# socom20/speech-cloner

Measured on AMD Instinct MI355X. Metric: mel frames/sec, higher is better.
Workload: dtype bf16; 1 GPU; full: STFT+mel front-end on batch 32 x 4 s @ 16 kHz (configs[1] input) -> 64 windows of 400 frames -> encoder (enc_14 weights) + decoder (hp/decoder_cfg_d.json sizes, random init), 64 windows per launch, independent steps pipelined over 10 HIP streams; batch=32, samples=64000, windows=64, model_dtype=bfloat16, streams=10, parallelism=utterance-sharded x1, no collective

## Files before the change

### include/vc_hip.h

```cpp
#ifndef VC_HIP_H
#define VC_HIP_H

#include <stddef.h>
#include <stdint.h>

#ifdef __cplusplus
extern "C" {
#endif

#define VC_OK 0
#define VC_ERR_INVALID 1
#define VC_ERR_HIP 2
#define VC_ERR_WORKSPACE 3
#define VC_ERR_UNSUPPORTED 4

#define VC_ABI_VERSION 7

int vc_version(void);
const char* vc_last_error(void);
const char* vc_target_arch(void);

int vc_set_option(const char* name, int value);
int vc_get_option(const char* name, int* value);

// ... 248 lines not shown
                           vc_vocoder_plan** out_plan);
void vc_vocoder_plan_destroy(vc_vocoder_plan* plan);
int32_t vc_vocoder_num_samples(const vc_vocoder_plan* plan, int32_t n_frames);
size_t vc_vocoder_workspace_bytes(const vc_vocoder_plan* plan, int32_t batch, int32_t max_frames, int32_t trace);

int vc_power_to_amp(const float* d_P, const int32_t* d_n_frames, int32_t batch, int32_t max_frames, int32_t n_bins,
                    float P_dB_norm_factor, float realse, float* d_amp, void* stream);

int vc_griffin_lim_f32(const vc_vocoder_plan* plan, const float* d_amp, const float* d_phase0,
                       const int32_t* d_n_frames, int32_t batch, int32_t max_frames, int32_t num_iters,
                       float* d_wav, int32_t wav_stride, float* d_trace, void* d_workspace, size_t workspace_bytes,
                       void* stream);

size_t vc_vocoder_workspace_bytes_momentum(const vc_vocoder_plan* plan, int32_t batch, int32_t max_frames,
                                           int32_t trace);
int vc_griffin_lim_momentum_f32(const vc_vocoder_plan* plan, const float* d_amp, const float* d_phase0,
                                const int32_t* d_n_frames, int32_t batch, int32_t max_frames, int32_t num_iters,
                                float momentum, float* d_wav, int32_t wav_stride, float* d_trace, void* d_workspace,
                                size_t workspace_bytes, void* stream);

int vc_inv_preemphasis_normalize(const vc_vocoder_plan* plan, float* d_wav, const int32_t* d_n_frames, int32_t batch,
                                 int32_t max_frames, int32_t wav_stride, float coeff, float mean_abs_amp_norm,
                                 void* stream);

int vc_highway_pack(const void* d_Bt, int32_t n_cols, int32_t H, void* d_packed, void* stream);
int vc_highway_chain(const void* d_X, int32_t M, int32_t H, int32_t ldx, int32_t n_layers,
                     const void* const* d_packed, const float* const* d_bias, void* d_Y, int32_t ldy,
                     const void* d_proj_packed, const float* d_proj_bias, int32_t n_proj, float* d_P, int32_t ldp,
                     void* stream);

#define VC_CBHG_FRONT_MAX_HIGHWAY 4
typedef struct vc_cbhg_front_desc {
    const void* d_x;
    int32_t x_f32, ldx;
    int32_t n_windows, T;
    int32_t n_features, prenet_units, width, n_banks, bank_filters, n_highway, gru_units;
    const void *d_pk_dense1, *d_pk_dense2, *d_pk_bank, *d_pk_proj1, *d_pk_proj2, *d_pk_gru;
    const void* d_pk_highway[VC_CBHG_FRONT_MAX_HIGHWAY];
    const float* d_coef;
    float* d_xproj;
    int32_t ldp;
} vc_cbhg_front_desc;
int vc_mfma_pack(const void* d_W, int32_t rows, int32_t K, int32_t ldw, int32_t chained, void* d_packed, void* stream);
int32_t vc_cbhg_front_coef_floats(void);
int vc_cbhg_front_supported(int32_t n_features, int32_t prenet_units, int32_t width, int32_t n_banks,
                            int32_t bank_filters, int32_t n_highway, int32_t gru_units, int32_t T);
int vc_cbhg_front(const vc_cbhg_front_desc* desc, void* stream);

int vc_prenet_chain_supported(int32_t cin_padded, int32_t units1, int32_t units2);
int vc_prenet_chain(const void* d_X, int32_t x_f32, int32_t M, int32_t ldx, int32_t cin_padded, int32_t units1, int32_t units2,
                    const void* d_pk1, const float* d_b1, const void* d_pk2, const float* d_b2, void* d_Y, int32_t ldy,
                    void* stream);

int vc_gather_rows(const void* d_src, const int64_t* d_index, const void* d_pad_row, int64_t n_rows,
                   int32_t row_bytes, void* d_dst, void* stream);

int vc_convert(const void* d_src, int32_t src_dtype, void* d_dst, int32_t dst_dtype, size_t n, void* stream);

int vc_cut_windows(const float* d_src, const int32_t* d_win_tab, const int32_t* d_n_frames, int32_t batch,
                   int32_t max_frames, int32_t n_windows, int32_t T, int32_t C, float* d_dst, void* stream);

int vc_compound_stitch(const void* d_src, int32_t src_dtype, const int32_t* d_utt_tab, int32_t batch, int32_t n_windows,
                       int32_t T, int32_t C, int32_t out_frames, float* d_dst, float* d_amp, float P_dB_norm_factor,
                       void* stream);

int vc_phase_init(const int32_t* d_n_frames, const int32_t* d_utt_id, int32_t batch, int32_t max_frames, int32_t n_bins,
                  int64_t seed, float* d_phase, void* stream);

size_t vc_phase_spsi_workspace_bytes(int32_t batch, int32_t max_frames, int32_t n_bins);
int vc_phase_spsi(const float* d_amp, const int32_t* d_n_frames, int32_t batch, int32_t max_frames, int32_t n_bins,
                  int32_t n_fft, int32_t hop, float* d_phase, void* d_workspace, size_t workspace_bytes, void* stream);

typedef struct vc_resample_plan vc_resample_plan;
int vc_resample_plan_create(int32_t up, int32_t down, int32_t half, const double* h_taps, vc_resample_plan** out_plan);
void vc_resample_plan_destroy(vc_resample_plan* plan);
int vc_resample_f32(const vc_resample_plan* plan, const float* d_in, const int32_t* d_lens_in, int32_t batch, int32_t max_in,
                    int32_t ld_in, float* d_out, int32_t max_out, int32_t ld_out, void* stream);

int vc_mel_cepstra(const void* d_mel, int32_t mel_dtype, int32_t rows, int32_t n_mels, const float* d_dct, int32_t n_coef,
                   float* d_cep, void* stream);
size_t vc_dtw_workspace_size(int32_t batch, int32_t max_a, int32_t max_b, int32_t want_path);
int vc_dtw_f32(const float* d_ca, const float* d_cb, const int32_t* d_len_a, const int32_t* d_len_b, int32_t batch,
               int32_t max_a, int32_t max_b, int32_t n_coef, float scale, int32_t band, int32_t want_path, float* d_total,
               int32_t* d_path_len, float* d_mcd, void* d_workspace, size_t workspace_bytes, void* stream);
int vc_dtw_backtrack(const void* d_workspace, size_t workspace_bytes, const int32_t* d_len_a, const int32_t* d_len_b,
                     const float* d_total, const int32_t* d_path_len, int32_t batch, int32_t max_a, int32_t max_b, int32_t* d_path,
                     void* stream);
int vc_frame_mcd_f32(const float* d_ca, const float* d_cb, const int32_t* d_len_a, const int32_t* d_len_b, int32_t batch,
                     int32_t max_a, int32_t max_b, int32_t n_coef, float scale, float* d_mcd, void* stream);

int vc_f0_yin_f32(const float* d_wav, const int32_t* d_lens, int32_t batch, int32_t max_len, int32_t ld, float sample_rate,
                  int32_t hop, int32_t frame_length, int32_t tau_min, int32_t tau_max, float threshold, float* d_f0,
                  float* d_aperiodicity, int32_t max_frames, void* stream);
int vc_f0_metrics_f32(const float* d_f0_a, const float* d_f0_b, const int32_t* d_len_a, const int32_t* d_len_b, int32_t batch,
                      int32_t max_a, int32_t max_b, const int32_t* d_path, const int32_t* d_path_len, int32_t max_path,
                      int32_t* d_counts, float* d_values, void* stream);

int vc_f0_candidates_f32(const float* d_wav, const int32_t* d_lens, int32_t batch, int32_t max_len, int32_t ld, float sample_rate,
                         int32_t hop, int32_t frame_length, int32_t tau_min, int32_t tau_max, float ceiling, int32_t n_cand,
                         float* d_f0, float* d_pitch, float* d_cost, int32_t* d_n, float* d_aperiodicity, int32_t max_frames,
                         void* stream);
int32_t vc_f0_viterbi_tile(void);
size_t vc_f0_viterbi_workspace_size(int32_t batch, int32_t max_frames, int32_t n_cand);
int vc_f0_viterbi_f32(const float* d_pitch, const float* d_cost, const int32_t* d_n, const int32_t* d_frames, int32_t batch,
                      int32_t max_frames, int32_t n_cand, float unvoiced_cost, float jump_cost, float switch_cost,
                      const float* d_cand_f0, int32_t* d_state, float* d_f0, float* d_total, void* d_workspace,
// ... 76 lines not shown
```

### speech-cloner_amd/_vc.py

```python
import contextlib
import ctypes as C
import os
import threading


_HERE = os.path.dirname(os.path.abspath(__file__))
LIB_PATH = os.environ.get('VC_LIB_PATH', os.path.join(_HERE, 'libvc_hip.so'))

VC_OK = 0
VC_ABI_VERSION = 7


class VCError(RuntimeError):
    pass


class FrontendCfg(C.Structure):
    _fields_ = [('sample_rate', C.c_int32), ('hop_length', C.c_int32), ('win_length', C.c_int32),
                ('n_fft', C.c_int32), ('n_mels', C.c_int32), ('n_mfcc', C.c_int32),
                ('pre_emphasis', C.c_float), ('mean_abs_amp_norm', C.c_float),
                ('mfcc_norm_factor', C.c_float), ('M_dB_norm_factor', C.c_float),
                ('P_dB_norm_factor', C.c_float),
                ('mfcc_normaleze_first_mfcc', C.c_int32), ('calc_mfcc_derivate', C.c_int32),
                ('clip_output', C.c_int32)]
# ... 118 lines not shown
    'vc_conv_gemm_workspace_bytes': (C.c_size_t, [C.POINTER(GemmDesc)]),
    'vc_conv_gemm': (C.c_int, [C.POINTER(GemmDesc), _P]),
    'vc_softmax_argmax': (C.c_int, [_P, C.c_int32, C.c_int32, C.c_int32, _P, C.c_int32, C.c_int32, _P, _P]),
    'vc_softmax_argmax_dual': (C.c_int, [_P, C.c_int32, C.c_int32, C.c_int32, _P, C.c_int32, _P, C.c_int32, _P, _P]),
    'vc_gru_workspace_bytes': (C.c_size_t, [C.c_int32, C.c_int32]),
    'vc_gru_bidir': (C.c_int, [_P, _P, _P, C.c_int32, C.c_int32, C.c_int32, C.c_int32, _P, C.c_int32, _P,
                               C.c_size_t, _P]),
    'vc_gru_form': (C.c_int32, [C.c_int32] * 4),
    'vc_gru_packed_bytes': (C.c_size_t, [C.c_int32] * 3),
    'vc_gru_pack': (C.c_int, [C.c_int32, _P, _P, C.c_int32, C.c_int32, _P, C.c_size_t, _P]),
    'vc_gru_bidir_packed': (C.c_int, [C.c_int32, _P, _P, C.c_size_t, C.c_int32, C.c_int32, C.c_int32, C.c_int32, _P, C.c_int32, _P]),
    'vc_lstm_bidir': (C.c_int, [_P, _P, _P, C.c_int32, C.c_int32, C.c_int32, C.c_int32, _P, C.c_int32, _P]),
    'vc_convert': (C.c_int, [_P, C.c_int32, _P, C.c_int32, C.c_size_t, _P]),
    'vc_conv_wgrad': (C.c_int, [C.POINTER(WgradDesc), _P]),
    'vc_transpose_pad': (C.c_int, [_P, C.c_int32, C.c_int32, C.c_int32, C.c_int32, _P, _P, C.c_int32, C.c_int32,
                                   C.c_int32, _P, C.c_int32, C.c_int32, C.c_int32, _P]),
    'vc_stats_workspace_floats': (C.c_size_t, [C.c_int32, C.c_int32]),
    'vc_bn_train_stats': (C.c_int, [_P, C.c_int32, C.c_int32, C.c_int32, _P, _P, _P, _P, C.c_float, C.c_float,
                                    _P, _P, _P, _P, _P, _P]),
    'vc_affine_act': (C.c_int, [_P, _P, _P, C.c_int32, _P, _P, C.c_size_t, C.c_int32, _P]),
    'vc_bn_backward': (C.c_int, [_P, _P, C.c_int32, C.c_int32, C.c_int32, C.c_int32, _P, _P, _P, _P, _P,
                                 C.c_int32, _P, _P, _P, _P, _P]),
    'vc_lstm_train_forward': (C.c_int, [_P, _P, _P, C.c_int32, C.c_int32, C.c_int32, _P, _P, _P, _P]),
    'vc_lstm_backward': (C.c_int, [_P, _P, _P, _P, _P, C.c_int32, C.c_int32, C.c_int32, _P, _P]),
    'vc_bn_post_routing': (C.c_int, [_P, C.c_int32, C.c_int32, C.c_int32, C.c_int32, _P, _P, _P, _P]),
    'vc_relu_dropout_backward': (C.c_int, [_P, _P, C.c_float, _P, C.c_size_t, _P]),
    'vc_highway_backward': (C.c_int, [_P, C.c_int32, _P, _P, C.c_int32, C.c_int32, _P, _P, _P]),
    'vc_col_sum': (C.c_int, [_P, C.c_int32, C.c_int32, C.c_int32, _P, C.c_int32, _P, _P]),
    'vc_fill': (C.c_int, [_P, C.c_float, C.c_size_t, _P]),
    'vc_weight_layouts': (C.c_int, [_P, C.c_int32, _P]),
    'vc_split16': (C.c_int, [_P, C.c_int32, C.c_int32, C.c_int32, C.c_int32, _P, _P, C.c_int32, C.c_int32, _P, _P, _P]),
    'vc_weights16': (C.c_int, [_P, C.c_int32, _P, C.c_int32, _P]),
    'vc_transpose_split16': (C.c_int, [_P, C.c_int32, C.c_int32, C.c_int32, C.c_int32, _P, _P, C.c_int32, C.c_int32, C.c_int32,
                                       C.c_int32, _P, _P, _P]),
    'vc_gemm16_workspace_bytes': (C.c_size_t, [C.c_int32, C.c_int32, C.c_int32]),
    'vc_gemm16': (C.c_int, [C.POINTER(Gemm16Desc), _P]),
    'vc_mx8_quantize': (C.c_int, [_P, C.c_int32, C.c_int32, C.c_int32, C.c_int32, _P, _P, _P]),
    'vc_mx8_conv_workspace_bytes': (C.c_size_t, [C.POINTER(Mx8ConvDesc)]),
    'vc_mx8_conv': (C.c_int, [C.POINTER(Mx8ConvDesc), _P]),
    'vc_axpby': (C.c_int, [_P, C.c_int32, C.c_float, _P, C.c_int32, C.c_float, _P, C.c_int32, C.c_int32, C.c_int32, _P]),
    'vc_mse_loss': (C.c_int, [_P, _P, C.c_size_t, C.c_float, _P, C.c_int32, C.c_int32, _P, _P, _P]),
    'vc_softmax_ce': (C.c_int, [_P, _P, C.c_int32, C.c_int32, C.c_int32, _P, C.c_int32, _P, _P, _P]),
    'vc_adam_step': (C.c_int, [_P, _P, _P, _P, C.c_size_t, C.c_float, C.c_float, C.c_float, C.c_float,
                               C.c_float, _P]),
    'vc_gru_train_forward': (C.c_int, [_P, _P, _P, C.c_int32, C.c_int32, C.c_int32, _P, _P, _P, _P]),
    'vc_gru_backward': (C.c_int, [_P, _P, _P, _P, _P, _P, _P, C.c_int32, C.c_int32, C.c_int32, _P, _P]),
    'vc_conv_gemm_epi_pool_supported': (C.c_int, [C.POINTER(GemmDesc)]),
    'vc_highway_pack': (C.c_int, [_P, C.c_int32, C.c_int32, _P, _P]),
    'vc_highway_chain': (C.c_int, [_P, C.c_int32, C.c_int32, C.c_int32, C.c_int32, C.POINTER(_P), C.POINTER(_P), _P, C.c_int32,
                                   _P, _P, C.c_int32, _P, C.c_int32, _P]),
    'vc_mfma_pack': (C.c_int, [_P, C.c_int32, C.c_int32, C.c_int32, C.c_int32, _P, _P]),
    'vc_prenet_chain_supported': (C.c_int, [C.c_int32] * 3),
    'vc_prenet_chain': (C.c_int, [_P, C.c_int32, C.c_int32, C.c_int32, C.c_int32, C.c_int32, C.c_int32, _P, _P, _P, _P, _P, C.c_int32, _P]),
    'vc_cbhg_front_coef_floats': (C.c_int32, []),
    'vc_cbhg_front_supported': (C.c_int, [C.c_int32] * 8),
    'vc_cbhg_front': (C.c_int, [C.POINTER(CbhgFrontDesc), _P]),
    'vc_gather_rows': (C.c_int, [_P, _P, _P, C.c_int64, C.c_int32, _P, _P]),
    'vc_vocoder_plan_create': (C.c_int, [C.c_int32, C.c_int32, C.c_int32, _P, C.POINTER(_P)]),
    'vc_vocoder_plan_destroy': (None, [_P]),
    'vc_vocoder_num_samples': (C.c_int32, [_P, C.c_int32]),
    'vc_vocoder_workspace_bytes': (C.c_size_t, [_P, C.c_int32, C.c_int32, C.c_int32]),
    'vc_power_to_amp': (C.c_int, [_P, _P, C.c_int32, C.c_int32, C.c_int32, C.c_float, C.c_float, _P, _P]),
    'vc_griffin_lim_f32': (C.c_int, [_P, _P, _P, _P, C.c_int32, C.c_int32, C.c_int32, _P, C.c_int32, _P, _P,
                                     C.c_size_t, _P]),
    'vc_vocoder_workspace_bytes_momentum': (C.c_size_t, [_P, C.c_int32, C.c_int32, C.c_int32]),
    'vc_griffin_lim_momentum_f32': (C.c_int, [_P, _P, _P, _P, C.c_int32, C.c_int32, C.c_int32, C.c_float, _P, C.c_int32,
                                              _P, _P, C.c_size_t, _P]),
    'vc_inv_preemphasis_normalize': (C.c_int, [_P, _P, _P, C.c_int32, C.c_int32, C.c_int32, C.c_float, C.c_float, _P]),
    'vc_cut_windows': (C.c_int, [_P, _P, _P, C.c_int32, C.c_int32, C.c_int32, C.c_int32, C.c_int32, _P, _P]),
    'vc_compound_stitch': (C.c_int, [_P, C.c_int32, _P, C.c_int32, C.c_int32, C.c_int32, C.c_int32, C.c_int32, _P, _P,
                                     C.c_float, _P]),
    'vc_phase_init': (C.c_int, [_P, _P, C.c_int32, C.c_int32, C.c_int32, C.c_int64, _P, _P]),
    'vc_phase_spsi_workspace_bytes': (C.c_size_t, [C.c_int32, C.c_int32, C.c_int32]),
    'vc_phase_spsi': (C.c_int, [_P, _P, C.c_int32, C.c_int32, C.c_int32, C.c_int32, C.c_int32, _P, _P, C.c_size_t, _P]),
    'vc_resample_plan_create': (C.c_int, [C.c_int32, C.c_int32, C.c_int32, _P, C.POINTER(_P)]),
    'vc_resample_plan_destroy': (None, [_P]),
    'vc_resample_f32': (C.c_int, [_P, _P, _P, C.c_int32, C.c_int32, C.c_int32, _P, C.c_int32, C.c_int32, _P]),
    'vc_mel_cepstra': (C.c_int, [_P, C.c_int32, C.c_int32, C.c_int32, _P, C.c_int32, _P, _P]),
    'vc_dtw_workspace_size': (C.c_size_t, [C.c_int32] * 4),
    'vc_dtw_f32': (C.c_int, [_P, _P, _P, _P, C.c_int32, C.c_int32, C.c_int32, C.c_int32, C.c_float, C.c_int32, C.c_int32, _P, _P, _P,
                             _P, C.c_size_t, _P]),
    'vc_dtw_backtrack': (C.c_int, [_P, C.c_size_t, _P, _P, _P, _P, C.c_int32, C.c_int32, C.c_int32, _P, _P]),
    'vc_frame_mcd_f32': (C.c_int, [_P, _P, _P, _P, C.c_int32, C.c_int32, C.c_int32, C.c_int32, C.c_float, _P, _P]),
    'vc_frame_energy_tile': (C.c_int, [C.c_int32, C.c_int32]),
    'vc_frame_energy_f32': (C.c_int, [_P, _P, C.c_int32, C.c_int32, C.c_int32, C.c_int32, C.c_int32, _P, C.c_int32, _P]),
    'vc_activity_mask': (C.c_int, [_P, _P, _P, C.c_int32, C.c_int32, C.c_int32, C.c_float, C.c_int32, C.c_int32, _P, _P]),
    'vc_mask_compact': (C.c_int, [_P, _P, C.c_int32, _P, _P, C.c_int32, C.c_int32, _P, _P, _P, _P, _P, _P]),
    'vc_compact_rows_f32': (C.c_int, [_P, C.c_int32, _P, C.c_int32, _P, C.c_int32, C.c_int32, _P, C.c_int32, _P]),
    'vc_path_map': (C.c_int, [_P, _P, C.c_int32, C.c_int32, _P, C.c_int32, _P, C.c_int32, _P, _P]),
    'vc_speech_gain_f32': (C.c_int, [_P, _P, C.c_int32, C.c_int32, C.c_int32, C.c_int32, _P, _P, C.c_int32, C.c_float, _P, _P]),
    'vc_scale_rows_f32': (C.c_int, [_P, _P, C.c_int32, C.c_int32, C.c_int32, _P, _P, _P]),
    'vc_ppg_metrics_f32': (C.c_int, [_P, _P, _P, _P, C.c_int32, C.c_int32, C.c_int32, C.c_int32, _P, _P, C.c_int32, _P, _P, _P, _P]),
    'vc_phn_segments_tile': (C.c_int, []),
    'vc_phn_segments': (C.c_int, [_P, _P, C.c_int32, C.c_int32, C.c_int32, C.c_int32, _P, _P, _P, _P, _P, _P]),
    'vc_edit_distance_rows': (C.c_int, []),
    'vc_edit_distance_workspace_bytes': (C.c_size_t, [C.c_int32] * 3),
    'vc_edit_distance_i32': (C.c_int, [_P, _P, _P, _P, C.c_int32, C.c_int32, C.c_int32, _P, _P, _P, C.c_size_t, _P]),
    'vc_gmm_tile_frames': (C.c_int, []),
    'vc_gmm_partitions': (C.c_int, [C.c_int32]),
    'vc_gmm_table_floats': (C.c_size_t, [C.c_int32] * 3),
    'vc_gmm_workspace_bytes': (C.c_size_t, [C.c_int32] * 3),
    'vc_spk_features_f32': (C.c_int, [_P, _P, _P, C.c_int32, C.c_int32, C.c_int32, C.c_int32, C.c_int32, _P, _P]),
    'vc_gmm_prepare_f32': (C.c_int, [_P, _P, _P, C.c_int32, C.c_int32, C.c_int32, _P, _P]),
    'vc_gmm_loglik_f32': (C.c_int, [_P, _P, C.c_int32, C.c_int32, C.c_int32, _P, C.c_int32, C.c_int32, _P, _P, _P, _P, _P]),
    'vc_gmm_score_f32': (C.c_int, [_P, _P, _P, _P, C.c_int32, C.c_int32, _P, _P, _P]),
    'vc_gmm_accumulate_f32': (C.c_int, [_P, _P, _P, _P, _P, C.c_int32, C.c_int32, C.c_int32, _P, C.c_int32, C.c_int32, C.c_int32,
# ... 101 lines not shown
```

### speech-cloner_amd/csrc/vc_api.hip

```cpp
#include <cstdarg>
#include <atomic>
#include <cstdio>
#include <cstring>
#include "vc_common.h"

namespace vc {

static thread_local char g_err[512] = "";

char* last_error_buf() { return g_err; }

int set_error(int code, const char* fmt, ...) {
    va_list ap;
    va_start(ap, fmt);
    vsnprintf(g_err, sizeof(g_err), fmt, ap);
    va_end(ap);
    return code;
}

static std::atomic<int> g_opt[OPT_COUNT];
static const struct { const char* name; Option id; } k_opts[] = {
    {"bank256", OPT_BANK256}, {"bank256_xcd", OPT_BANK256_XCD}, {"conv256", OPT_CONV256},
    {"conv256_min_k", OPT_CONV256_MINK}, {"conv256_wm", OPT_CONV256_WM}, {"proj256", OPT_PROJ256}, {"proj256_split", OPT_PROJ256_SPLIT},
    {"wgrad_xcd", OPT_WGRAD_XCD}, {"gru_mfma", OPT_GRU_MFMA}, {"fe_fused", OPT_FE_FUSED},
    {"fe_fused_spin", OPT_FE_FUSED_SPIN}, {"gru_train_resident", OPT_GRU_TRAIN_RESIDENT},
    {"prenet_lds", OPT_PRENET_LDS}, {"cbhg_front_mi", OPT_CBHG_FRONT_MI}, {"gemm16_split", OPT_GEMM16_SPLIT},
    {"f32_f16x3", OPT_F32_F16X3}, {"gru_f32_wide", OPT_GRU_F32_WIDE},
};
static struct OptInit { OptInit() { for (auto& o : g_opt) o.store(-1); } } g_opt_init;

int opt(Option o) { return g_opt[o].load(std::memory_order_relaxed); }

static __global__ void zero_words_kernel(unsigned* __restrict__ p, size_t n) {
    for (size_t i = (size_t)blockIdx.x * blockDim.x + threadIdx.x; i < n; i += (size_t)gridDim.x * blockDim.x) p[i] = 0u;
}

hipError_t zero_async(void* d_p, size_t bytes, hipStream_t st) {
    if (bytes % 4) return hipErrorInvalidValue;
    const size_t n = bytes / 4;
    if (n == 0) return hipSuccess;
    const size_t blocks = (n + 255) / 256;
    hipLaunchKernelGGL(zero_words_kernel, dim3((unsigned)(blocks < 1024 ? blocks : 1024)), dim3(256), 0, st,
                       static_cast<unsigned*>(d_p), n);
    return hipGetLastError();
}

}

extern "C" {

int vc_set_option(const char* name, int value) {
    VC_REQUIRE(name, "vc_set_option: NULL name");
    for (const auto& o : vc::k_opts)
        if (!std::strcmp(o.name, name)) {
            vc::g_opt[o.id].store(value);
            return VC_OK;
        }
    return vc::set_error(VC_ERR_INVALID, "vc_set_option: unknown option %s", name);
}

int vc_get_option(const char* name, int* value) {
    VC_REQUIRE(name && value, "vc_get_option: NULL argument");
    for (const auto& o : vc::k_opts)
        if (!std::strcmp(o.name, name)) { *value = vc::g_opt[o.id].load(); return VC_OK; }
    return vc::set_error(VC_ERR_INVALID, "vc_get_option: unknown option %s", name);
}

int vc_version(void) { return VC_ABI_VERSION; }
const char* vc_last_error(void) { return vc::last_error_buf(); }
const char* vc_target_arch(void) { return "gfx950"; }

}
```

### speech-cloner_amd/csrc/vc_cbhg_small.hip

```cpp
#include "vc_device.h"
#include <cstdlib>

using vc::f32x16, vc::f32x4, vc::bf16x8, vc::bf16x4;

namespace {

constexpr int CS_C = 40;
constexpr int CS_PITCH = 2 * CS_C;
constexpr int CS_GF = 4, CS_GB = 8;
constexpr int cs_tile_bytes(int mi) { return (CS_GF + 32 * mi + CS_GB) * CS_PITCH; }
constexpr int CS_RED_PITCH = 176;
constexpr int cs_red_bytes(int mi) { return 32 * mi * CS_RED_PITCH; }
constexpr int CS_MAX_HW = 4;

struct CbhgSmallArgs {
    const void* X; int32_t x_f32, ldx;
    int32_t n_windows, T, TF, tiles_per_win, n_hw;
    const bf16x8 *pk_d1, *pk_d2, *pk_bank, *pk_p1, *pk_p2, *pk_x;
    const bf16x8* pk_hw[CS_MAX_HW];
    const float* coef;
    float* P; int32_t ldp;
};

__device__ __forceinline__ f32x16 zero16() {
// ... 509 lines not shown
        for (int s = 0; s < KS1; ++s) {
            const int f = tl * KS1 + s;
            if (f % CH == 0) publish(f / CH);
            acc = mfma(frag(f), xb[s], acc);
        }
#pragma unroll
        for (int q = 0; q < 4; ++q) {
            const f32x4 bb = *reinterpret_cast<const f32x4*>(bias + 32 * tl + 8 * q + 4 * lh);
#pragma unroll
            for (int e = 0; e < 4; ++e) y1[tl][q][e] = (__bf16)fmaxf(acc[4 * q + e] + bb[e], 0.0f);
        }
    }
#pragma unroll
    for (int tl = 0; tl < NT2; ++tl) {
        f32x16 acc = zero16();
#pragma unroll
        for (int s = 0; s < KS2; ++s) {
            const int f = NF1 + tl * KS2 + s;
            if (f % CH == 0) publish(f / CH);
            acc = mfma(frag(f), chain<NT1>(y1, s), acc);
        }
#pragma unroll
        for (int q = 0; q < 4; ++q) {
            const f32x4 bb = *reinterpret_cast<const f32x4*>(bias + U1 + 32 * tl + 8 * q + 4 * lh);
            bf16x4 o;
#pragma unroll
            for (int e = 0; e < 4; ++e) o[e] = (__bf16)fmaxf(acc[4 * q + e] + bb[e], 0.0f);
            *reinterpret_cast<bf16x4*>(tile + li * PITCH + (32 * tl + 8 * q + 4 * lh) * 2) = o;
        }
    }
    wave_lds_fence();
    constexpr int CPR = U2 / 8;
    for (int idx = lane; idx < 32 * CPR; idx += 64) {
        const int r = idx / CPR, c = idx - r * CPR;
        if (m0 + r < a.M)
            *reinterpret_cast<bf16x8*>(a.Y + (size_t)(m0 + r) * a.ldy + c * 8) = *reinterpret_cast<const bf16x8*>(tile + r * PITCH + c * 16);
    }
}

template <int CINP, int U1, int U2> int launch_prenet_chain(const PrenetArgs& a, hipStream_t st) {
    constexpr int LDS = 4 * 32 * (U2 * 2 + 16);
    constexpr int LDS_SHARED = LDS + 3 * 16 * 1024 + (U1 + U2) * 4;
    if (int rc = vc::allow_dynamic_lds<prenet_chain_kernel<CINP, U1, U2>>(LDS)) return rc;
    if (int rc = vc::allow_dynamic_lds<prenet_chain_lds_kernel<CINP, U1, U2>>(LDS_SHARED)) return rc;
    const dim3 grid((unsigned)((a.M + 127) / 128));
    if (vc::opt(vc::OPT_PRENET_LDS) != 0)
        hipLaunchKernelGGL((prenet_chain_lds_kernel<CINP, U1, U2>), grid, dim3(256), LDS_SHARED, st, a);
    else
        hipLaunchKernelGGL((prenet_chain_kernel<CINP, U1, U2>), grid, dim3(256), LDS, st, a);
    VC_HIP_CHECK(hipGetLastError());
    return VC_OK;
}

__global__ void __launch_bounds__(256)
mfma_pack_kernel(const __bf16* W, int rows, int K, int ldw, int chained, int ntiles, int nks, __bf16* out) {
    const int total = ntiles * nks * 64 * 8;
    for (int idx = blockIdx.x * 256 + threadIdx.x; idx < total; idx += gridDim.x * 256) {
        int r = idx;
        const int e = r & 7; r >>= 3;
        const int lane = r & 63; r >>= 6;
        const int s = r % nks, tl = r / nks;
        const int row = 32 * tl + (lane & 31), h = lane >> 5;
        const int col = chained ? 32 * (s >> 1) + 8 * (2 * (s & 1) + (e >> 2)) + 4 * h + (e & 3) : 16 * s + 8 * h + e;
        out[idx] = (row < rows && col < K) ? W[(size_t)row * ldw + col] : (__bf16)0.0f;
    }
}

constexpr int cbhg_small_lds(int mi) { return cbhg_small_lds_tiles(mi) + CO_TOTAL * 4; }

template <int MI> int launch_cbhg_small(const CbhgSmallArgs& a, int n_windows, hipStream_t st) {
    if (int rc = vc::allow_dynamic_lds<cbhg_small_kernel<6, 80, 80, MI>>(cbhg_small_lds(MI))) return rc;
    hipLaunchKernelGGL((cbhg_small_kernel<6, 80, 80, MI>), dim3((unsigned)(n_windows * a.tiles_per_win)), dim3(256),
                       cbhg_small_lds(MI), st, a);
    VC_HIP_CHECK(hipGetLastError());
    return VC_OK;
}

}

extern "C" {

int vc_mfma_pack(const void* d_W, int32_t rows, int32_t K, int32_t ldw, int32_t chained, void* d_packed, void* stream) {
    VC_REQUIRE(d_W && d_packed && rows > 0 && K > 0 && ldw >= K, "vc_mfma_pack: bad argument");
    const int ntiles = (rows + 31) / 32, nks = (K + 15) / 16;
    hipLaunchKernelGGL(mfma_pack_kernel, dim3(64), dim3(256), 0, static_cast<hipStream_t>(stream),
                       static_cast<const __bf16*>(d_W), rows, K, ldw, chained, ntiles, nks, static_cast<__bf16*>(d_packed));
    VC_HIP_CHECK(hipGetLastError());
    return VC_OK;
}

int vc_prenet_chain_supported(int32_t cin_padded, int32_t units1, int32_t units2) {
    return (cin_padded == 64 && units1 == 256 && units2 == 128) || (cin_padded == 80 && units1 == 512 && units2 == 256);
}

int vc_prenet_chain(const void* d_X, int32_t x_f32, int32_t M, int32_t ldx, int32_t cin_padded, int32_t units1, int32_t units2,
                    const void* d_pk1, const float* d_b1, const void* d_pk2, const float* d_b2, void* d_Y, int32_t ldy,
                    void* stream) {
    VC_REQUIRE(d_X && d_pk1 && d_b1 && d_pk2 && d_b2 && d_Y && M > 0, "vc_prenet_chain: NULL argument or M <= 0");
    VC_REQUIRE(vc_prenet_chain_supported(cin_padded, units1, units2), "vc_prenet_chain: unsupported shape %d -> %d -> %d", cin_padded, units1, units2);
    VC_REQUIRE(ldx >= cin_padded && ldx % (x_f32 ? 4 : 8) == 0 && ldy >= units2 && ldy % 8 == 0, "vc_prenet_chain: leading dimensions must keep rows 16-byte aligned and cover them");
    VC_REQUIRE(((reinterpret_cast<uintptr_t>(d_X) | reinterpret_cast<uintptr_t>(d_Y) | reinterpret_cast<uintptr_t>(d_pk1) |
                 reinterpret_cast<uintptr_t>(d_pk2) | reinterpret_cast<uintptr_t>(d_b1) | reinterpret_cast<uintptr_t>(d_b2)) & 15) == 0,
               "vc_prenet_chain: operands must be 16-byte aligned");
    PrenetArgs a;
    a.X = d_X; a.x_f32 = x_f32 ? 1 : 0; a.M = M; a.ldx = ldx;
    a.pk1 = static_cast<const bf16x8*>(d_pk1); a.pk2 = static_cast<const bf16x8*>(d_pk2);
    a.b1 = d_b1; a.b2 = d_b2; a.Y = static_cast<__bf16*>(d_Y); a.ldy = ldy;
    hipStream_t st = static_cast<hipStream_t>(stream);
    return cin_padded == 64 ? launch_prenet_chain<64, 256, 128>(a, st) : launch_prenet_chain<80, 512, 256>(a, st);
}

int32_t vc_cbhg_front_coef_floats(void) { return CO_TOTAL; }

int vc_cbhg_front_supported(int32_t n_features, int32_t prenet_units, int32_t width, int32_t n_banks, int32_t bank_filters,
                            int32_t n_highway, int32_t gru_units, int32_t T) {
    return n_features == 80 && prenet_units == 80 && width == CS_C && n_banks == 6 && bank_filters == 128 &&
           n_highway >= 0 && n_highway <= CS_MAX_HW && gru_units == CS_C && T >= 8;
}

int vc_cbhg_front(const vc_cbhg_front_desc* d, void* stream) {
    VC_REQUIRE(d, "vc_cbhg_front: NULL descriptor");
    VC_REQUIRE(vc_cbhg_front_supported(d->n_features, d->prenet_units, d->width, d->n_banks, d->bank_filters, d->n_highway,
                                       d->gru_units, d->T),
               "vc_cbhg_front: unsupported shape (features %d, prenet %d, width %d, banks %d x %d, highway %d, gru %d)",
               d->n_features, d->prenet_units, d->width, d->n_banks, d->bank_filters, d->n_highway, d->gru_units);
    VC_REQUIRE(d->d_x && d->d_xproj && d->n_windows > 0 && d->ldx >= d->n_features && d->ldp >= 6 * d->gru_units,
               "vc_cbhg_front: NULL tensor or bad leading dimension");
    VC_REQUIRE((d->ldx * (d->x_f32 ? 4 : 2)) % 16 == 0 && d->ldp % 4 == 0 &&
                   ((reinterpret_cast<uintptr_t>(d->d_x) | reinterpret_cast<uintptr_t>(d->d_xproj)) & 15) == 0,
               "vc_cbhg_front: rows of x / xproj must be 16-byte aligned");
    const void* ptrs[] = {d->d_pk_dense1, d->d_pk_dense2, d->d_pk_bank, d->d_pk_proj1, d->d_pk_proj2, d->d_pk_gru, d->d_coef};
    for (const void* p : ptrs) VC_REQUIRE(p && (reinterpret_cast<uintptr_t>(p) & 15) == 0, "vc_cbhg_front: NULL or misaligned weight pointer");
    CbhgSmallArgs a = {};
    a.X = d->d_x; a.x_f32 = d->x_f32; a.ldx = d->ldx;
    a.n_windows = d->n_windows; a.T = d->T; a.n_hw = d->n_highway;
    constexpr int HL = 2 + (6 - 1) / 2;
    a.pk_d1 = static_cast<const bf16x8*>(d->d_pk_dense1); a.pk_d2 = static_cast<const bf16x8*>(d->d_pk_dense2);
    a.pk_bank = static_cast<const bf16x8*>(d->d_pk_bank); a.pk_p1 = static_cast<const bf16x8*>(d->d_pk_proj1);
    a.pk_p2 = static_cast<const bf16x8*>(d->d_pk_proj2); a.pk_x = static_cast<const bf16x8*>(d->d_pk_gru);
    a.coef = d->d_coef;
    for (int l = 0; l < d->n_highway; ++l) {
        VC_REQUIRE(d->d_pk_highway[l] && (reinterpret_cast<uintptr_t>(d->d_pk_highway[l]) & 15) == 0, "vc_cbhg_front: highway layer %d weights NULL or misaligned", l);
        a.pk_hw[l] = static_cast<const bf16x8*>(d->d_pk_highway[l]);
    }
    a.P = d->d_xproj; a.ldp = d->ldp;
    const int mi = vc::opt(vc::OPT_CBHG_FRONT_MI) == 4 ? 4 : 2;
    const int maxtf = 32 * mi - HL - 6;
    a.tiles_per_win = (d->T + maxtf - 1) / maxtf;
    a.TF = (d->T + a.tiles_per_win - 1) / a.tiles_per_win;
    return mi == 4 ? launch_cbhg_small<4>(a, d->n_windows, static_cast<hipStream_t>(stream))
                   : launch_cbhg_small<2>(a, d->n_windows, static_cast<hipStream_t>(stream));
}

}
```

### speech-cloner_amd/csrc/vc_common.h

```cpp
#pragma once
#include <hip/hip_runtime.h>
#include <cstdarg>
#include <cstdio>
#include "vc_hip.h"

namespace vc {

char* last_error_buf();
int set_error(int code, const char* fmt, ...);

#define VC_HIP_CHECK(expr)                                                                   \
    do {                                                                                     \
        hipError_t _e = (expr);                                                              \
        if (_e != hipSuccess)                                                                \
            return vc::set_error(VC_ERR_HIP, "%s failed: %s (%s:%d)", #expr,                 \
                                 hipGetErrorString(_e), __FILE__, __LINE__);                 \
    } while (0)

#define VC_REQUIRE(cond, ...)                                                                \
    do {                                                                                     \
        if (!(cond)) return vc::set_error(VC_ERR_INVALID, __VA_ARGS__);                      \
    } while (0)

constexpr int WAVE = 64;

enum Option {
    OPT_BANK256 = 0,
    OPT_BANK256_XCD,
    OPT_CONV256,
    OPT_CONV256_MINK,
    OPT_CONV256_WM,
    OPT_PROJ256,
    OPT_PROJ256_SPLIT,
    OPT_WGRAD_XCD,
    OPT_GRU_MFMA,
    OPT_FE_FUSED,
    OPT_FE_FUSED_SPIN,
    OPT_PRENET_LDS,
    OPT_GRU_TRAIN_RESIDENT,
    OPT_CBHG_FRONT_MI,
    OPT_GRU_F32_WIDE,
    OPT_F32_F16X3,
    OPT_GEMM16_SPLIT,
    OPT_COUNT
};
int opt(Option o);

hipError_t zero_async(void* d_p, size_t bytes, hipStream_t st);

#if defined(__HIPCC__)
template <int CTRL, int ROW_MASK>
__device__ __forceinline__ float dpp_move(float identity, float v) {
    return __int_as_float(__builtin_amdgcn_update_dpp(__float_as_int(identity), __float_as_int(v), CTRL, ROW_MASK, 0xF, false));
}
#define VC_WAVE_REDUCE(OP, ID)                                                                  \
    v = OP(v, dpp_move<0xB1, 0xF>(ID, v));                             \
    v = OP(v, dpp_move<0x4E, 0xF>(ID, v));                             \
    v = OP(v, dpp_move<0x141, 0xF>(ID, v));                                \
    v = OP(v, dpp_move<0x140, 0xF>(ID, v));          \
    v = OP(v, dpp_move<0x142, 0xA>(ID, v));                 \
    v = OP(v, dpp_move<0x143, 0xC>(ID, v));                 \
    return __int_as_float(__builtin_amdgcn_readlane(__float_as_int(v), 63));
__device__ __forceinline__ float vc_addf(float a, float b) { return a + b; }
__device__ __forceinline__ float wave_sum(float v) { VC_WAVE_REDUCE(vc_addf, 0.0f) }
__device__ __forceinline__ float wave_max(float v) { VC_WAVE_REDUCE(fmaxf, -3.402823466e38f) }
__device__ __forceinline__ float highway_gate(float hpre, float tpre, float x) {
    const float hv = fmaxf(hpre, 0.0f);
    const float e = __builtin_amdgcn_exp2f(tpre * -1.4426950408889634f);
    const float tv = __builtin_amdgcn_rcpf(1.0f + e);
    return fmaf(tv, hv - x, x);
}
__device__ __forceinline__ float wave_min(float v) { VC_WAVE_REDUCE(fminf, 3.402823466e38f) }
#undef VC_WAVE_REDUCE
#endif

}
```

### speech-cloner_amd/modules.py

```python
import contextlib
import ctypes as C
import math
import threading

import numpy as np

import _vc
import mx8

OPTIONS = {'prenet_chain': True,
           'highway_chain': True,
           'cbhg_front': True}


def apply_options(d):
    for k, v in (d or {}).items():
        if k in OPTIONS:
            OPTIONS[k] = bool(v)
        else:
            _vc.set_option(k, int(v))

BN_EPS = 1e-3
BN_DECAY = 0.999
BANK_FILTERS = 128
# ... 275 lines not shown
            bias[64 * q + 32:64 * q + 32 + (hi - lo)] = b2[lo:hi]
        return bt.to(store.dtype).contiguous(), bias
    return store.cached(('highway', scope), build)


def _prep_gru(store, scope, cin, H):
    w = {}
    for d in ('fw', 'bw'):
        s = '{}/bidirectional_rnn/{}/gru_cell'.format(scope, d)
        w[d] = (store.get(s + '/gates/kernel', (cin + H, 2 * H), 'glorot'),
                store.get(s + '/gates/bias', (2 * H,), 1.0),
                store.get(s + '/candidate/kernel', (cin + H, H), 'glorot'),
                store.get(s + '/candidate/bias', (H,), 0.0))

    def build():
        torch = _torch()
        btx = torch.cat([torch.cat([w[d][0][:cin].t(), w[d][2][:cin].t()], 0) for d in ('fw', 'bw')], 0)
        bx = torch.cat([torch.cat([w[d][1], w[d][3]], 0) for d in ('fw', 'bw')], 0)
        wh = [torch.cat([w[d][0][cin:], w[d][2][cin:]], 1).contiguous().to(store.dtype) for d in ('fw', 'bw')]
        return btx.contiguous().to(store.dtype), bx.contiguous(), wh[0], wh[1]
    return store.cached(('gru', scope), build)


def _prep_gru_uni(store, scope, cin, H):
    s = '{}/rnn/gru_cell'.format(scope)
    wg = store.get(s + '/gates/kernel', (cin + H, 2 * H), 'glorot')
    bg = store.get(s + '/gates/bias', (2 * H,), 1.0)
    wc = store.get(s + '/candidate/kernel', (cin + H, H), 'glorot')
    bc = store.get(s + '/candidate/bias', (H,), 0.0)

    def build():
        torch = _torch()
        one = torch.cat([wg[:cin].t(), wc[:cin].t()], 0)
        b1 = torch.cat([bg, bc], 0)
        wh = torch.cat([wg[cin:], wc[cin:]], 1).contiguous().to(store.dtype)
        return torch.cat([one, one], 0).contiguous().to(store.dtype), torch.cat([b1, b1], 0).contiguous(), wh
    return store.cached(('gru_uni', scope), build)


def dense(inputs, units, activation_fn=None, name='dense', bias_init=0.0, out_f32=False, in_features=None):
    torch = _torch()
    store = _store()
    x = _as3(inputs)
    N_, T_, Cx = x.shape
    scope = _scope(name)
    cin = Cx if in_features is None else in_features
    kname = scope + '/kernel'
    if kname in store.vars:
        cin = store.vars[kname].shape[0]
    bt, b = _prep_dense(store, scope, cin, units, bias_init)
    if Cx != _pad8(cin):
        raise ValueError(' - ERROR, dense {}: input width {} does not match kernel rows {}'.format(scope, Cx, cin))
    out = torch.empty((N_, T_, units), dtype=torch.float32 if out_f32 else store.dtype, device=x.device)
    act = {None: _vc.ACT_NONE, 'relu': _vc.ACT_RELU, 'sigmoid': _vc.ACT_SIGMOID, 'tanh': _vc.ACT_TANH}[activation_fn]
    gemm_launch(x, N_ * T_, T_, Cx, Cx, units, [(bt, Cx, 1, 0, 0)], out, units, store.vc_dtype,
                epi_shift=b, act=act, out_f32=out_f32)
    return out


def bn(inputs, is_training=True, activation_fn=None, scope="bn", reuse=None):
    if is_training:
        raise NotImplementedError(' - ERROR, bn: training-mode batch statistics are fused into the training step')
    torch = _torch()
    store = _store()
    x = _as3(inputs)
    N_, T_, C_ = x.shape
    s, sh = _prep_bn(store, _scope(scope), C_)
    eye = store.cached(('eye', C_), lambda: torch.eye(C_, dtype=store.dtype, device=store.device))
    out = torch.empty_like(x)
    act = {None: _vc.ACT_NONE, 'relu': _vc.ACT_RELU}[activation_fn]
    gemm_launch(x, N_ * T_, T_, C_, C_, C_, [(eye, C_, 1, 0, 0)], out, C_, store.vc_dtype,
                epi_scale=s, epi_shift=sh, act=act)
    return out


def _f32_split_ok(store):
    return store.dtype == _torch().float32 and _vc.get_option('f32_f16x3') != 0


def _mx8_ok(store):
    return getattr(store, 'mx8', False)


def conv1d(inputs, filters=None, size=1, rate=1, padding="SAME", use_bias=False, activation_fn=None,
           scope="conv1d", reuse=None, bn_scope=None, residual=None, pool_input=False):
    if rate != 1 or padding.upper() != "SAME" or use_bias:
        raise NotImplementedError(' - ERROR, conv1d: only rate=1, padding=SAME, use_bias=False are used by the reference')
    torch = _torch()
    store = _store()
    if isinstance(inputs, mx8.MxTensor):
        N_, T_, Cin = inputs.shape
        filters = Cin if filters is None else filters
        if not (_mx8_ok(store) and mx8.conv_supported(Cin, filters, size) and residual is None and not pool_input):
            raise ValueError(' - ERROR, conv1d {}: an MX-FP8 input needs mxfp8 mode, a multiple of 128 filters, no '
                             'residual and no input pooling'.format(_scope(scope)))
        with variable_scope(scope):
            kscope = _scope()
            store.get(kscope + '/conv1d/kernel', (size, Cin, filters), 'glorot')
        if bn_scope is not None:
            s, sh = _prep_bn(store, _scope(bn_scope), filters)
        else:
            s = store.cached(('ones', filters), lambda: torch.ones(filters, dtype=torch.float32, device=store.device))
            sh = store.cached(('zeros', filters), lambda: torch.zeros(filters, dtype=torch.float32, device=store.device))
        packed = store.cached(('mx8conv', kscope, bn_scope), lambda: mx8.pack_kernel(store.vars[kscope + '/conv1d/kernel']))
        act = {None: _vc.ACT_NONE, 'relu': _vc.ACT_RELU}[activation_fn]
        return mx8.conv(inputs, packed, size, filters, s, sh, act)
# ... 453 lines not shown
```

Measured before the change: 14.14 million frames/s.

## Add specialized MFMA dense-rows kernel for small-output f32 projection layers

Adds a dedicated bf16 MFMA kernel for dense layers with no activation that write f32 output, for the shapes 256->80, 512->201 and 80->61. Each wave keeps its 32 input rows in registers. Pre-packed weight fragments are streamed into a triple-buffered LDS ring with async global-to-LDS loads, and outputs are staged through LDS so stores are coalesced. It replaces the generic gemm_launch path for these output projections, aiming to cut launch and tiling overhead on narrow N. In exchange it adds a cached packed weight copy, an option gate, and a large LDS footprint that allows one block per CU.

```diff
diff --git a/include/vc_hip.h b/include/vc_hip.h
--- a/include/vc_hip.h
+++ b/include/vc_hip.h
@@ -324,6 +324,10 @@
                     const void* d_pk1, const float* d_b1, const void* d_pk2, const float* d_b2, void* d_Y, int32_t ldy,
                     void* stream);
 
+int vc_dense_rows_supported(int32_t K, int32_t N);
+int vc_dense_rows(const void* d_X, int32_t M, int32_t ldx, int32_t K, int32_t N, const void* d_packed, const float* d_bias,
+                  float* d_Y, int32_t ldy, void* stream);
+
 int vc_gather_rows(const void* d_src, const int64_t* d_index, const void* d_pad_row, int64_t n_rows,
                    int32_t row_bytes, void* d_dst, void* stream);
 
diff --git a/speech-cloner_amd/_vc.py b/speech-cloner_amd/_vc.py
--- a/speech-cloner_amd/_vc.py
+++ b/speech-cloner_amd/_vc.py
@@ -194,6 +194,8 @@
     'vc_mfma_pack': (C.c_int, [_P, C.c_int32, C.c_int32, C.c_int32, C.c_int32, _P, _P]),
     'vc_prenet_chain_supported': (C.c_int, [C.c_int32] * 3),
     'vc_prenet_chain': (C.c_int, [_P, C.c_int32, C.c_int32, C.c_int32, C.c_int32, C.c_int32, C.c_int32, _P, _P, _P, _P, _P, C.c_int32, _P]),
+    'vc_dense_rows_supported': (C.c_int, [C.c_int32] * 2),
+    'vc_dense_rows': (C.c_int, [_P, C.c_int32, C.c_int32, C.c_int32, C.c_int32, _P, _P, _P, C.c_int32, _P]),
     'vc_cbhg_front_coef_floats': (C.c_int32, []),
     'vc_cbhg_front_supported': (C.c_int, [C.c_int32] * 8),
     'vc_cbhg_front': (C.c_int, [C.POINTER(CbhgFrontDesc), _P]),
diff --git a/speech-cloner_amd/csrc/vc_api.hip b/speech-cloner_amd/csrc/vc_api.hip
--- a/speech-cloner_amd/csrc/vc_api.hip
+++ b/speech-cloner_amd/csrc/vc_api.hip
@@ -25,7 +25,7 @@
     {"wgrad_xcd", OPT_WGRAD_XCD}, {"gru_mfma", OPT_GRU_MFMA}, {"fe_fused", OPT_FE_FUSED},
     {"fe_fused_spin", OPT_FE_FUSED_SPIN}, {"gru_train_resident", OPT_GRU_TRAIN_RESIDENT},
     {"prenet_lds", OPT_PRENET_LDS}, {"cbhg_front_mi", OPT_CBHG_FRONT_MI}, {"gemm16_split", OPT_GEMM16_SPLIT},
-    {"f32_f16x3", OPT_F32_F16X3}, {"gru_f32_wide", OPT_GRU_F32_WIDE},
+    {"f32_f16x3", OPT_F32_F16X3}, {"gru_f32_wide", OPT_GRU_F32_WIDE}, {"dense_rows", OPT_DENSE_ROWS},
 };
 static struct OptInit { OptInit() { for (auto& o : g_opt) o.store(-1); } } g_opt_init;
 
diff --git a/speech-cloner_amd/csrc/vc_cbhg_small.hip b/speech-cloner_amd/csrc/vc_cbhg_small.hip
--- a/speech-cloner_amd/csrc/vc_cbhg_small.hip
+++ b/speech-cloner_amd/csrc/vc_cbhg_small.hip
@@ -585,6 +585,100 @@
     return VC_OK;
 }
 
+struct DenseRowsArgs {
+    const __bf16* X; int32_t M, ldx;
+    const bf16x8* pk;
+    const float* b;
+    float* Y;
+};
+
+template <int K, int N>
+__global__ void __launch_bounds__(256, 1)
+dense_rows_lds_kernel(DenseRowsArgs a) {
+    static_assert(K % 16 == 0, "shape");
+    constexpr int KS = K / 16, NT = (N + 31) / 32, NF = NT * KS, CH = 16, NC = (NF + CH - 1) / CH;
+    constexpr int TILE = 32 * N * 4;
+    constexpr int O_W = 4 * TILE, O_B = O_W + 3 * CH * 1024;
+    extern __shared__ __attribute__((aligned(16))) char smem[];
+    const int tid = threadIdx.x, lane = tid & 63;
+    const int w = __builtin_amdgcn_readfirstlane(tid >> 6);
+    const int li = lane & 31, lh = lane >> 5;
+    const int m0 = blockIdx.x * 128 + 32 * w;
+    const int row = min(m0 + li, a.M - 1);
+    float* const tile = reinterpret_cast<float*>(smem + w * TILE);
+    char* const wbuf = smem + O_W;
+    float* const bias = reinterpret_cast<float*>(smem + O_B);
+
+    auto request = [&](int c) {
+        char* dst = wbuf + (c % 3) * CH * 1024 + w * 4096;
+#pragma unroll
+        for (int u = 0; u < 4; ++u) vc::glds16(a.pk + (size_t)min(c * CH + w * 4 + u, NF - 1) * 64 + lane, dst + u * 1024);
+    };
+
+    bf16x8 xb[KS];
+    {
+        const __bf16* xr = a.X + (size_t)row * a.ldx + 8 * lh;
+#pragma unroll
+        for (int s = 0; s < KS; ++s) xb[s] = *reinterpret_cast<const bf16x8*>(xr + 16 * s);
+    }
+    for (int i = tid; i < 32 * NT; i += 256) bias[i] = i < N ? a.b[i] : 0.0f;
+    asm volatile("s_waitcnt vmcnt(0)" ::: "memory");
+    request(0);
+    if (NC > 1) request(1);
+    auto publish = [&](int c) {
+        if (c + 1 < NC) asm volatile("s_waitcnt vmcnt(4)" ::: "memory");
+        else asm volatile("s_waitcnt vmcnt(0)" ::: "memory");
+        __syncthreads();
+        if (c + 2 < NC) request(c + 2);
+    };
+    auto frag = [&](int f) -> bf16x8 {
+        return *reinterpret_cast<const bf16x8*>(wbuf + ((f / CH) % 3) * CH * 1024 + (f % CH) * 1024 + lane * 16);
+    };
+
+#pragma unroll
+    for (int tl = 0; tl < NT; ++tl) {
+        f32x16 acc = zero16();
+#pragma unroll
+        for (int s = 0; s < KS; ++s) {
+            const int f = tl * KS + s;
+            if (f % CH == 0) publish(f / CH);
+            acc = mfma(frag(f), xb[s], acc);
+        }
+#pragma unroll
+        for (int q = 0; q < 4; ++q) {
+            const int c0 = 32 * tl + 8 * q + 4 * lh;
+            const f32x4 bb = *reinterpret_cast<const f32x4*>(bias + c0);
+            f32x4 o;
+#pragma unroll
+            for (int e = 0; e < 4; ++e) o[e] = acc[4 * q + e] + bb[e];
+            if constexpr (N % 4 == 0) {
+                if (c0 < N) *reinterpret_cast<f32x4*>(tile + li * N + c0) = o;
+            } else {
+#pragma unroll
+                for (int e = 0; e < 4; ++e)
+                    if (c0 + e < N) tile[li * N + c0 + e] = o[e];
+            }
+        }
+    }
+    wave_lds_fence();
+    const int rows = min(32, a.M - m0);
+    if (rows <= 0) return;
+    const int total = rows * N, nv = total >> 2;
+    float* const y = a.Y + (size_t)m0 * N;
+    for (int idx = lane; idx < nv; idx += 64)
+        reinterpret_cast<f32x4*>(y)[idx] = reinterpret_cast<const f32x4*>(tile)[idx];
+    if (lane < (total & 3)) y[4 * nv + lane] = tile[4 * nv + lane];
+}
+
+template <int K, int N> int launch_dense_rows(const DenseRowsArgs& a, hipStream_t st) {
+    constexpr int LDS = 4 * 32 * N * 4 + 3 * 16 * 1024 + ((N + 31) / 32) * 32 * 4;
+    static_assert(LDS <= 160 * 1024, "one block's tiles, chunk buffers and bias fit the CU's LDS");
+    if (int rc = vc::allow_dynamic_lds<dense_rows_lds_kernel<K, N>>(LDS)) return rc;
+    hipLaunchKernelGGL((dense_rows_lds_kernel<K, N>), dim3((unsigned)((a.M + 127) / 128)), dim3(256), LDS, st, a);
+    VC_HIP_CHECK(hipGetLastError());
+    return VC_OK;
+}
+
 __global__ void __launch_bounds__(256)
 mfma_pack_kernel(const __bf16* W, int rows, int K, int ldw, int chained, int ntiles, int nks, __bf16* out) {
     const int total = ntiles * nks * 64 * 8;
@@ -641,6 +735,26 @@
     a.b1 = d_b1; a.b2 = d_b2; a.Y = static_cast<__bf16*>(d_Y); a.ldy = ldy;
     hipStream_t st = static_cast<hipStream_t>(stream);
     return cin_padded == 64 ? launch_prenet_chain<64, 256, 128>(a, st) : launch_prenet_chain<80, 512, 256>(a, st);
+}
+
+int vc_dense_rows_supported(int32_t K, int32_t N) {
+    return (K == 256 && N == 80) || (K == 512 && N == 201) || (K == 80 && N == 61);
+}
+
+int vc_dense_rows(const void* d_X, int32_t M, int32_t ldx, int32_t K, int32_t N, const void* d_packed, const float* d_bias,
+                  float* d_Y, int32_t ldy, void* stream) {
+    VC_REQUIRE(d_X && d_packed && d_bias && d_Y && M > 0, "vc_dense_rows: NULL argument or M <= 0");
+    VC_REQUIRE(vc_dense_rows_supported(K, N), "vc_dense_rows: unsupported shape %d -> %d", K, N);
+    VC_REQUIRE(ldx >= K && ldx % 8 == 0 && ldy == N, "vc_dense_rows: ldx must be a multiple of 8 and >= K, ldy must equal N (dense output rows)");
+    VC_REQUIRE(((reinterpret_cast<uintptr_t>(d_X) | reinterpret_cast<uintptr_t>(d_Y) | reinterpret_cast<uintptr_t>(d_packed)) & 15) == 0 &&
+                   (reinterpret_cast<uintptr_t>(d_bias) & 3) == 0, "vc_dense_rows: X / Y / packed weights must be 16-byte aligned");
+    DenseRowsArgs a;
+    a.X = static_cast<const __bf16*>(d_X); a.M = M; a.ldx = ldx;
+    a.pk = static_cast<const bf16x8*>(d_packed); a.b = d_bias; a.Y = d_Y;
+    hipStream_t st = static_cast<hipStream_t>(stream);
+    if (K == 256) return launch_dense_rows<256, 80>(a, st);
+    if (K == 512) return launch_dense_rows<512, 201>(a, st);
+    return launch_dense_rows<80, 61>(a, st);
 }
 
 int32_t vc_cbhg_front_coef_floats(void) { return CO_TOTAL; }
diff --git a/speech-cloner_amd/csrc/vc_common.h b/speech-cloner_amd/csrc/vc_common.h
--- a/speech-cloner_amd/csrc/vc_common.h
+++ b/speech-cloner_amd/csrc/vc_common.h
@@ -42,6 +42,7 @@
     OPT_GRU_F32_WIDE,
     OPT_F32_F16X3,
     OPT_GEMM16_SPLIT,
+    OPT_DENSE_ROWS,
     OPT_COUNT
 };
 int opt(Option o);
diff --git a/speech-cloner_amd/modules.py b/speech-cloner_amd/modules.py
--- a/speech-cloner_amd/modules.py
+++ b/speech-cloner_amd/modules.py
@@ -351,6 +351,12 @@
     if Cx != _pad8(cin):
         raise ValueError(' - ERROR, dense {}: input width {} does not match kernel rows {}'.format(scope, Cx, cin))
     out = torch.empty((N_, T_, units), dtype=torch.float32 if out_f32 else store.dtype, device=x.device)
+    if (out_f32 and activation_fn is None and store.dtype == torch.bfloat16 and x.dtype == torch.bfloat16 and x.is_contiguous()
+            and _vc.lib().vc_dense_rows_supported(Cx, units) and _vc.get_option('dense_rows') != 0):
+        pk = store.cached(('dense_rows_pk', scope), lambda: _mfma_pack(bt, units, Cx, 0))
+        _vc.check(_vc.lib().vc_dense_rows(x.data_ptr(), N_ * T_, Cx, Cx, units, pk.data_ptr(), b.data_ptr(), out.data_ptr(),
+                                          units, _vc.current_stream()))
+        return out
     act = {None: _vc.ACT_NONE, 'relu': _vc.ACT_RELU, 'sigmoid': _vc.ACT_SIGMOID, 'tanh': _vc.ACT_TANH}[activation_fn]
     gemm_launch(x, N_ * T_, T_, Cx, Cx, units, [(bt, Cx, 1, 0, 0)], out, units, store.vc_dtype,
                 epi_shift=b, act=act, out_f32=out_f32)
```

Result: no change. 14.27 million frames/s (median of 6 runs) (+1.0%).
